# kserve/kserve

Hardware: AMD Instinct MI355X
Metric: output tok/s, llama-3-8b /v1/completions decode (higher is better)
Workload: dtype bfloat16; 1 GPU; model=llama-3-8b, global_batch=1536, seq_len=512, parallelism=dp1, kv_block_size=16, hipgraph=True, kv_cache_dtype=auto

## Files before the change

### kserve_amd/ops/csrc/attention_decode.hip

```cpp
#include "common.h"
#include "mfma_layouts.h"

#define NEG_INF (-1e30f)

namespace {

constexpr int PAGE = 16;
constexpr int NWAVES = 4;

typedef __bf16 bf16x2v_t __attribute__((ext_vector_type(2)));

template <int D, int HPW, int OCC = 1, bool PB = false, bool D2 = false,
          bool V4 = false, bool MQ = false>
__global__ __launch_bounds__(256, OCC) void paged_attention_kernel(
    short* __restrict__ out,
    const short* __restrict__ q,
    const short* __restrict__ k_cache,
    const short* __restrict__ v_cache,
    const int* __restrict__ block_tables,
    const int* __restrict__ context_lens,
    const float scale,
    const int num_kv_heads,
    const int group,
    const int max_blocks,
    const long q_row_stride,
    const int n_splits,
    float* __restrict__ part_out,
    float* __restrict__ part_ml,
    const int window
) {
  constexpr int ACC = D / 64;
  const int kv_head = blockIdx.x;
  const int seq = blockIdx.y;
  const int split = blockIdx.z;
  const int ctx = context_lens[seq];
  if (ctx <= 0) return;
  const int num_heads = num_kv_heads * group;
  const int lane = threadIdx.x & 63;
  const int wave = threadIdx.x >> 6;
  const int tok = lane >> 2;
  const int part = lane & 3;
  __shared__ float p_bc[NWAVES][PAGE];

  const int nblocks = (ctx + PAGE - 1) / PAGE;
  const int wstart = (window > 0 && ctx > window) ? ctx - window : 0;
  const int first_blk = wstart / PAGE;
  const int blocks_per_split =
      (nblocks - first_blk + n_splits - 1) / n_splits;
  const int blk_lo = first_blk + split * blocks_per_split;
  const int blk_hi = min(nblocks, blk_lo + blocks_per_split);
  if (blk_lo >= blk_hi) {
    if (n_splits > 1 && threadIdx.x < (unsigned)group) {
      const int h = kv_head * group + threadIdx.x;
      float* ml = part_ml + (((long)seq * num_heads + h) * n_splits + split) * 2;
      ml[0] = NEG_INF;
      ml[1] = 0.f;
    }
    return;
  }

  constexpr int QFRAG = D / 4;
  float q_frag[HPW][D2 ? 1 : QFRAG];
  bf16x2v_t q_pk[HPW][D2 ? QFRAG / 2 : 1];
  int heads[HPW];
  bool hact[HPW];
  bool any_active = false;
  const int nw = blockDim.x >> 6;
#pragma unroll
  for (int h = 0; h < HPW; ++h) {
    const int head = kv_head * group + wave + h * nw;
    heads[h] = head;
    hact[h] = (wave + h * nw) < group;
    any_active |= hact[h];
    if (hact[h]) {
      const short* qp =
          q + (long)seq * q_row_stride + (long)head * D + part * QFRAG;
      if constexpr (D2) {
        const bf16x2v_t* qp2 = reinterpret_cast<const bf16x2v_t*>(qp);
#pragma unroll
        for (int j = 0; j < QFRAG / 2; ++j) q_pk[h][j] = qp2[j];
      } else {
#pragma unroll
        for (int j = 0; j < QFRAG; ++j)
          q_frag[h][j] = bf16_bits_to_float(qp[j]);
      }
    }
  }

  bf16x8_t q_mf[MQ ? D / 32 : 1];
  if constexpr (MQ) {
    const short* qb = q + (long)seq * q_row_stride + (long)heads[0] * D;
#pragma unroll
    for (int ki = 0; ki < D / 32; ++ki)
      q_mf[ki] = *reinterpret_cast<const bf16x8_t*>(
          qb + ki * 32 + ((lane >> 4) << 3));
  }

  float m[HPW], l[HPW];
  float acc[HPW][ACC];
  float acc8[V4 ? 8 : 1];
#pragma unroll
  for (int h = 0; h < HPW; ++h) {
    m[h] = NEG_INF;
    l[h] = 0.f;
#pragma unroll
    for (int a = 0; a < ACC; ++a) acc[h][a] = 0.f;
  }
#pragma unroll
  for (int a = 0; a < (V4 ? 8 : 1); ++a) acc8[a] = 0.f;

  if (!any_active) return;
  const int bt_base = (int)((long)seq * max_blocks);
  for (int bi = blk_lo; bi < blk_hi; ++bi) {
    const int block_id = block_tables[bt_base + bi];
    const short* page =
        k_cache + (((long)block_id * num_kv_heads + kv_head) * PAGE) * D;
    const short8_t* kp =
        reinterpret_cast<const short8_t*>(page + tok * D + part * QFRAG);
    const int gtok = bi * PAGE + tok;
    const bool tok_valid = gtok < ctx && gtok >= wstart;
    const short* vpage =
        v_cache + (((long)block_id * num_kv_heads + kv_head) * PAGE) * D;

    if constexpr (MQ && HPW == 1 && V4) {
      short8_t vwide4[4];
      const int vdim = (lane & 15) * 8;
      const int vtok4 = lane >> 4;
#pragma unroll
      for (int q4 = 0; q4 < 4; ++q4)
        vwide4[q4] = *reinterpret_cast<const short8_t*>(
            vpage + (q4 * 4 + vtok4) * D + vdim);
      f32x4_t cfrag = f32x4_t{0.f, 0.f, 0.f, 0.f};
#pragma unroll
      for (int ki = 0; ki < D / 32; ++ki) {
        const bf16x8_t bk = *reinterpret_cast<const bf16x8_t*>(
            page + (lane & 15) * D + ki * 32 + ((lane >> 4) << 3));
        cfrag = mfma16x16x32(q_mf[ki], bk, cfrag);
      }
      const int mytok = bi * PAGE + (lane & 15);
      const bool my_valid =
          lane < 16 && mytok < ctx && mytok >= wstart;
      float s = my_valid ? cfrag[0] * scale : NEG_INF;
      float tmax = s;
#pragma unroll
      for (int off = 1; off < 64; off <<= 1)
        tmax = fmaxf(tmax, __shfl_xor(tmax, off, 64));
      const float m_new = fmaxf(m[0], tmax);
      const float rescale = __expf(m[0] - m_new);
      const float p = (s > NEG_INF) ? __expf(s - m_new) : 0.f;
      float psum = p;
#pragma unroll
      for (int off = 1; off < 64; off <<= 1)
        psum += __shfl_xor(psum, off, 64);
      l[0] = l[0] * rescale + psum;
      m[0] = m_new;
      if (lane < 16) p_bc[wave][lane] = p;
      asm volatile("s_waitcnt lgkmcnt(0)");
#pragma unroll
      for (int a = 0; a < 8; ++a) acc8[a] *= rescale;
#pragma unroll
      for (int q4 = 0; q4 < 4; ++q4) {
// ... 563 lines not shown
  const int split = blockIdx.z;
  const int ctx = context_lens[seq];
  if (ctx <= 0) return;
  const int num_heads = num_kv_heads * GROUP;
  const int lane = threadIdx.x & 63;
  const int wave = threadIdx.x >> 6;
  const int tok = lane >> 2;
  const int part = lane & 3;

  const int nblocks = (ctx + PAGE - 1) / PAGE;
  const int wstart = (window > 0 && ctx > window) ? ctx - window : 0;
  const int first_blk = wstart / PAGE;
  const int blocks_per_split =
      (nblocks - first_blk + n_splits - 1) / n_splits;
  const int blk_lo = first_blk + split * blocks_per_split;
  const int blk_hi = min(nblocks, blk_lo + blocks_per_split);

  __shared__ float lds_ml[NWAVES][GROUP][2];
  __shared__ float lds_acc[NWAVES][GROUP][64 * ACC];

  if (blk_lo >= blk_hi) {
    if (n_splits > 1 && threadIdx.x < (unsigned)GROUP) {
      const int h = kv_head * GROUP + threadIdx.x;
      float* ml = part_ml + (((long)seq * num_heads + h) * n_splits + split) * 2;
      ml[0] = NEG_INF;
      ml[1] = 0.f;
    }
    return;
  }

  const short8_t* qrows[GROUP];
#pragma unroll
  for (int g = 0; g < GROUP; ++g) {
    qrows[g] = reinterpret_cast<const short8_t*>(
        q + (long)seq * q_row_stride + (long)(kv_head * GROUP + g) * D +
        part * QFRAG);
  }

  float m[GROUP], l[GROUP], acc[GROUP][ACC];
#pragma unroll
  for (int g = 0; g < GROUP; ++g) {
    m[g] = NEG_INF;
    l[g] = 0.f;
#pragma unroll
    for (int a = 0; a < ACC; ++a) acc[g][a] = 0.f;
  }

  const int bt_base = (int)((long)seq * max_blocks);
  for (int bi = blk_lo + wave; bi < blk_hi; bi += NWAVES) {
    const int block_id = block_tables[bt_base + bi];
    const long pbase = (((long)block_id * num_kv_heads + kv_head) * PAGE) * D;
    const short8_t* kp =
        reinterpret_cast<const short8_t*>(k_cache + pbase + tok * D + part * QFRAG);
    short8_t kreg[QFRAG / 8];
#pragma unroll
    for (int c = 0; c < QFRAG / 8; ++c) kreg[c] = kp[c];
    const short* vpage = v_cache + pbase;
    unsigned int vreg[PAGE];
#pragma unroll
    for (int t = 0; t < PAGE; ++t) {
      if constexpr (ACC == 2) {
        vreg[t] =
            *reinterpret_cast<const unsigned int*>(vpage + t * D + lane * ACC);
      } else {
        vreg[t] = (unsigned short)*(vpage + t * D + lane);
      }
    }
    const int gtok = bi * PAGE + tok;
    const bool tok_valid = gtok < ctx && gtok >= wstart;
#pragma unroll 1
    for (int g = 0; g < GROUP; ++g) {
      float s = 0.f;
#pragma unroll
      for (int c = 0; c < QFRAG / 8; ++c) {
        const short8_t qv = qrows[g][c];
#pragma unroll
        for (int j = 0; j < 8; ++j)
          s += bf16_bits_to_float(qv[j]) * bf16_bits_to_float(kreg[c][j]);
      }
      s = group_reduce_sum<4>(s);
      s = tok_valid ? s * scale : NEG_INF;
      const float tmax = wave_reduce_max(s);
      const float m_new = fmaxf(m[g], tmax);
      const float rescale = __expf(m[g] - m_new);
      const float p = (s > NEG_INF) ? __expf(s - m_new) : 0.f;
      const float psum = wave_reduce_sum(part == 0 ? p : 0.f);
      l[g] = l[g] * rescale + psum;
#pragma unroll
      for (int a = 0; a < ACC; ++a) acc[g][a] *= rescale;
      m[g] = m_new;
#pragma unroll
      for (int t = 0; t < PAGE; ++t) {
        const float pt = __shfl(p, t * 4, 64);
        if constexpr (ACC == 2) {
          acc[g][0] += pt * bf16_bits_to_float((short)(vreg[t] & 0xFFFF));
          acc[g][1] += pt * bf16_bits_to_float((short)(vreg[t] >> 16));
        } else {
          acc[g][0] += pt * bf16_bits_to_float((short)vreg[t]);
        }
      }
    }
  }

#pragma unroll
  for (int g = 0; g < GROUP; ++g) {
    if (lane == 0) {
      lds_ml[wave][g][0] = m[g];
      lds_ml[wave][g][1] = l[g];
    }
#pragma unroll
    for (int a = 0; a < ACC; ++a)
      lds_acc[wave][g][lane * ACC + a] = acc[g][a];
  }
  __syncthreads();
  for (int g = wave; g < GROUP; g += NWAVES) {
    float m_all = NEG_INF;
#pragma unroll
    for (int w = 0; w < NWAVES; ++w) m_all = fmaxf(m_all, lds_ml[w][g][0]);
    float l_all = 0.f;
    float a_all[ACC];
#pragma unroll
    for (int a = 0; a < ACC; ++a) a_all[a] = 0.f;
#pragma unroll
    for (int w = 0; w < NWAVES; ++w) {
      const float wgt = __expf(lds_ml[w][g][0] - m_all);
      l_all += wgt * lds_ml[w][g][1];
#pragma unroll
      for (int a = 0; a < ACC; ++a)
        a_all[a] += wgt * lds_acc[w][g][lane * ACC + a];
    }
    const int head = kv_head * GROUP + g;
    if (n_splits == 1) {
      const float inv_l = (l_all > 0.f) ? 1.f / l_all : 0.f;
      short* op = out + ((long)seq * num_heads + head) * D + lane * ACC;
#pragma unroll
      for (int a = 0; a < ACC; ++a)
        op[a] = float_to_bf16_bits(a_all[a] * inv_l);
    } else {
      float* po = part_out +
                  (((long)seq * num_heads + head) * n_splits + split) * D +
                  lane * ACC;
#pragma unroll
      for (int a = 0; a < ACC; ++a) po[a] = a_all[a];
      if (lane == 0) {
        float* ml =
            part_ml + (((long)seq * num_heads + head) * n_splits + split) * 2;
        ml[0] = m_all;
        ml[1] = l_all;
      }
    }
  }
}

template <int D>
__global__ void paged_attention_reduce_kernel(
    short* __restrict__ out,
    const float* __restrict__ part_out,
    const float* __restrict__ part_ml,
    const long total_sh, const int n_splits) {
  constexpr int ACC = D / 64;
  const long sh = blockIdx.x * (long)(blockDim.x >> 6) + (threadIdx.x >> 6);
  const int lane = threadIdx.x & 63;
  if (sh >= total_sh) return;
  const float* ml_base = part_ml + sh * n_splits * 2;
  float m = NEG_INF;
  for (int sp = 0; sp < n_splits; ++sp) m = fmaxf(m, ml_base[sp * 2]);
  float l = 0.f;
  float acc[ACC];
#pragma unroll
  for (int a = 0; a < ACC; ++a) acc[a] = 0.f;
  for (int sp = 0; sp < n_splits; ++sp) {
    const float ms = ml_base[sp * 2];
    const float ls = ml_base[sp * 2 + 1];
    if (ls <= 0.f || ms <= NEG_INF) continue;
    const float w = __expf(ms - m);
    l += ls * w;
    const float* po = part_out + (sh * n_splits + sp) * D + lane * ACC;
#pragma unroll
    for (int a = 0; a < ACC; ++a) acc[a] += w * po[a];
  }
  const float inv_l = (l > 0.f) ? 1.f / l : 0.f;
  short* op = out + sh * D + lane * ACC;
#pragma unroll
  for (int a = 0; a < ACC; ++a) op[a] = float_to_bf16_bits(acc[a] * inv_l);
}

}


namespace {
inline hipError_t launch_split_reduce(void* out, void* part_out,
                                      void* part_ml, int num_seqs,
                                      int num_heads, int head_dim,
                                      int n_splits, hipStream_t stream) {
  if (n_splits <= 1) return hipSuccess;
  const long sh = (long)num_seqs * num_heads;
  const int wpb = 4;
  dim3 rgrid((unsigned)((sh + wpb - 1) / wpb));
  if (head_dim == 128) {
    hipLaunchKernelGGL((paged_attention_reduce_kernel<128>), rgrid,
                       dim3(wpb * 64), 0, stream, (short*)out,
                       (const float*)part_out, (const float*)part_ml, sh,
                       n_splits);
  } else {
    hipLaunchKernelGGL((paged_attention_reduce_kernel<64>), rgrid,
                       dim3(wpb * 64), 0, stream, (short*)out,
                       (const float*)part_out, (const float*)part_ml, sh,
                       n_splits);
  }
  HIP_CHECK_KERNEL();
  return hipSuccess;
}
}

extern "C" hipError_t ks_paged_attention_decode_fp8(
    void* out, const void* q, const void* k_cache, const void* v_cache,
    const void* block_tables, const void* context_lens, float scale,
    int num_seqs, int num_heads, int num_kv_heads, int head_dim,
    int max_blocks, int block_size, long q_row_stride, int n_splits,
    void* part_out, void* part_ml, int window, hipStream_t stream) {
  if (block_size != PAGE || head_dim != 128) return hipErrorInvalidValue;
  const int group = num_heads / num_kv_heads;
  if (group > NWAVES) return hipErrorInvalidValue;
  if (n_splits < 1) n_splits = 1;
  dim3 grid(num_kv_heads, num_seqs, n_splits);
  static const bool cvtb = [] {
    const char* e = getenv("KS_FP8_CVTB");
    return e == nullptr || e[0] != '0';
  }();
  if (cvtb) {
    hipLaunchKernelGGL((paged_attention_fp8_kernel<128, true>), grid,
                       dim3(256), 0, stream, (short*)out, (const short*)q,
                       (const unsigned char*)k_cache,
                       (const unsigned char*)v_cache,
                       (const int*)block_tables, (const int*)context_lens,
                       scale, num_kv_heads, group, max_blocks, q_row_stride,
                       n_splits, (float*)part_out, (float*)part_ml, window);
  } else {
    hipLaunchKernelGGL((paged_attention_fp8_kernel<128, false>), grid,
                       dim3(256), 0, stream, (short*)out, (const short*)q,
                       (const unsigned char*)k_cache,
                       (const unsigned char*)v_cache,
                       (const int*)block_tables, (const int*)context_lens,
                       scale, num_kv_heads, group, max_blocks, q_row_stride,
                       n_splits, (float*)part_out, (float*)part_ml, window);
  }
  HIP_CHECK_KERNEL();
  return launch_split_reduce(out, part_out, part_ml, num_seqs, num_heads,
                             head_dim, n_splits, stream);
}

extern "C" hipError_t ks_paged_attention_decode(
    void* out, const void* q, const void* k_cache, const void* v_cache,
    const void* block_tables, const void* context_lens, float scale,
    int num_seqs, int num_heads, int num_kv_heads, int head_dim,
    int max_blocks, int block_size, long q_row_stride, int n_splits,
    void* part_out, void* part_ml, int window, hipStream_t stream) {
  if (block_size != PAGE) return hipErrorInvalidValue;
  const int group = num_heads / num_kv_heads;
  const int hpw = (group + NWAVES - 1) / NWAVES;
  if (hpw > 2) return hipErrorInvalidValue;
  if (n_splits < 1) n_splits = 1;
  dim3 grid(num_kv_heads, num_seqs, n_splits);
  dim3 block(256);

  static const bool use_ws = [] {
    const char* e = getenv("KS_ATTN_WS");
    return e != nullptr && e[0] == '1';
  }();
  const bool pow2_group =
      group == 1 || group == 2 || group == 4 || group == 8;
  if (use_ws && pow2_group && head_dim == 128) {
#define LAUNCH_WS(GG)                                                       \
  hipLaunchKernelGGL((paged_attention_ws_kernel<128, GG>), grid, block, 0,  \
                     stream, (short*)out, (const short*)q,                  \
                     (const short*)k_cache, (const short*)v_cache,          \
                     (const int*)block_tables, (const int*)context_lens,    \
                     scale, num_kv_heads, max_blocks, q_row_stride,         \
                     n_splits, (float*)part_out, (float*)part_ml, window)
    if (group == 1) LAUNCH_WS(1);
    else if (group == 2) LAUNCH_WS(2);
    else if (group == 4) LAUNCH_WS(4);
    else LAUNCH_WS(8);
#undef LAUNCH_WS
    HIP_CHECK_KERNEL();
    return launch_split_reduce(out, part_out, part_ml, num_seqs, num_heads,
                               head_dim, n_splits, stream);
  }

  static const bool use_h2 = [] {
    const char* e = getenv("KS_ATTN_H2");
    return e != nullptr && e[0] == '1';
  }();
  if (use_h2 && group == 4 && head_dim == 128) {
    hipLaunchKernelGGL((paged_attention_kernel<128, 2>), grid, dim3(128), 0,
                       stream, (short*)out, (const short*)q,
                       (const short*)k_cache, (const short*)v_cache,
                       (const int*)block_tables, (const int*)context_lens,
                       scale, num_kv_heads, group, max_blocks, q_row_stride,
                       n_splits, (float*)part_out, (float*)part_ml, window);
    HIP_CHECK_KERNEL();
    return launch_split_reduce(out, part_out, part_ml, num_seqs, num_heads,
                               head_dim, n_splits, stream);
  }

  static const bool use_mq = [] {
    const char* e = getenv("KS_ATTN_MQ");
    return e != nullptr && e[0] == '1';
  }();
  if (use_mq && hpw == 1 && head_dim == 128) {
    hipLaunchKernelGGL(
        (paged_attention_kernel<128, 1, 1, true, false, true, true>), grid,
        block, 0, stream, (short*)out, (const short*)q,
        (const short*)k_cache, (const short*)v_cache,
        (const int*)block_tables, (const int*)context_lens, scale,
        num_kv_heads, group, max_blocks, q_row_stride, n_splits,
        (float*)part_out, (float*)part_ml, window);
    HIP_CHECK_KERNEL();
    return launch_split_reduce(out, part_out, part_ml, num_seqs, num_heads,
                               head_dim, n_splits, stream);
  }

  static const bool use_u2 = [] {
    const char* e = getenv("KS_ATTN_U2");
    return e != nullptr && e[0] == '1';
  }();
  if (use_u2 && hpw == 1 && head_dim == 128) {
    hipLaunchKernelGGL((paged_attention_u2_kernel<128>), grid, block, 0,
                       stream, (short*)out, (const short*)q,
                       (const short*)k_cache, (const short*)v_cache,
                       (const int*)block_tables, (const int*)context_lens,
                       scale, num_kv_heads, group, max_blocks, q_row_stride,
                       n_splits, (float*)part_out, (float*)part_ml, window);
    HIP_CHECK_KERNEL();
    return launch_split_reduce(out, part_out, part_ml, num_seqs, num_heads,
                               head_dim, n_splits, stream);
  }
  static const int occ = [] {
    const char* e = getenv("KS_ATTN_OCC");
    return e ? atoi(e) : 0;
  }();
  static const bool use_pb = [] {
    const char* e = getenv("KS_ATTN_PB");
    return e == nullptr || e[0] != '0';
  }();
  static const int v4_mode = [] {
    const char* e = getenv("KS_ATTN_V4");
    return e ? (e[0] == '1' ? 1 : 0) : -1;
  }();
  const bool use_v4 =
      v4_mode == 1 || (v4_mode == -1 && num_seqs > 128);
  static const bool v4_d2 = [] {
    const char* e = getenv("KS_ATTN_V4D2");
    return e != nullptr && e[0] == '1';
  }();
  if (use_v4 && hpw == 1 && head_dim == 128) {
    if (v4_d2) {
      hipLaunchKernelGGL(
          (paged_attention_kernel<128, 1, 1, true, true, true>), grid, block,
          0, stream, (short*)out, (const short*)q, (const short*)k_cache,
          (const short*)v_cache, (const int*)block_tables,
          (const int*)context_lens, scale, num_kv_heads, group, max_blocks,
          q_row_stride, n_splits, (float*)part_out, (float*)part_ml, window);
    } else {
      hipLaunchKernelGGL(
          (paged_attention_kernel<128, 1, 1, true, false, true>), grid,
          block, 0, stream, (short*)out, (const short*)q,
          (const short*)k_cache, (const short*)v_cache,
          (const int*)block_tables, (const int*)context_lens, scale,
          num_kv_heads, group, max_blocks, q_row_stride, n_splits,
          (float*)part_out, (float*)part_ml, window);
    }
    HIP_CHECK_KERNEL();
    return launch_split_reduce(out, part_out, part_ml, num_seqs, num_heads,
                               head_dim, n_splits, stream);
  }
  static const int d2_mode = [] {
    const char* e = getenv("KS_ATTN_D2");
    return e ? (e[0] == '1' ? 1 : 0) : -1;
  }();
  const bool use_d2 =
      d2_mode == 1 || (d2_mode == -1 && num_seqs <= 128);
  if (use_d2 && hpw == 1 && head_dim == 128) {
    hipLaunchKernelGGL((paged_attention_kernel<128, 1, 1, true, true>), grid,
                       block, 0, stream, (short*)out, (const short*)q,
                       (const short*)k_cache, (const short*)v_cache,
                       (const int*)block_tables, (const int*)context_lens,
                       scale, num_kv_heads, group, max_blocks, q_row_stride,
                       n_splits, (float*)part_out, (float*)part_ml, window);
    HIP_CHECK_KERNEL();
    return launch_split_reduce(out, part_out, part_ml, num_seqs, num_heads,
                               head_dim, n_splits, stream);
  }
  if (use_pb && hpw == 1 && head_dim == 128) {
    hipLaunchKernelGGL((paged_attention_kernel<128, 1, 1, true>), grid, block,
                       0, stream, (short*)out, (const short*)q,
                       (const short*)k_cache, (const short*)v_cache,
                       (const int*)block_tables, (const int*)context_lens,
                       scale, num_kv_heads, group, max_blocks, q_row_stride,
                       n_splits, (float*)part_out, (float*)part_ml, window);
    HIP_CHECK_KERNEL();
    return launch_split_reduce(out, part_out, part_ml, num_seqs, num_heads,
                               head_dim, n_splits, stream);
  }
  if (occ >= 5 && hpw == 1 && head_dim == 128) {
    if (occ >= 6) {
      hipLaunchKernelGGL((paged_attention_kernel<128, 1, 6>), grid, block, 0,
                         stream, (short*)out, (const short*)q,
                         (const short*)k_cache, (const short*)v_cache,
                         (const int*)block_tables, (const int*)context_lens,
                         scale, num_kv_heads, group, max_blocks, q_row_stride,
                         n_splits, (float*)part_out, (float*)part_ml, window);
    } else {
      hipLaunchKernelGGL((paged_attention_kernel<128, 1, 5>), grid, block, 0,
                         stream, (short*)out, (const short*)q,
                         (const short*)k_cache, (const short*)v_cache,
                         (const int*)block_tables, (const int*)context_lens,
                         scale, num_kv_heads, group, max_blocks, q_row_stride,
                         n_splits, (float*)part_out, (float*)part_ml, window);
    }
    HIP_CHECK_KERNEL();
    return launch_split_reduce(out, part_out, part_ml, num_seqs, num_heads,
                               head_dim, n_splits, stream);
  }
#define LAUNCH_PA(DD, HH)                                                  \
  hipLaunchKernelGGL((paged_attention_kernel<DD, HH>), grid, block, 0,     \
                     stream, (short*)out, (const short*)q,                 \
                     (const short*)k_cache, (const short*)v_cache,         \
                     (const int*)block_tables, (const int*)context_lens,   \
                     scale, num_kv_heads, group, max_blocks, q_row_stride, \
                     n_splits, (float*)part_out, (float*)part_ml, window)
  if (head_dim == 128) {
    if (hpw == 1) LAUNCH_PA(128, 1);
    else LAUNCH_PA(128, 2);
  } else if (head_dim == 64) {
    if (hpw == 1) LAUNCH_PA(64, 1);
    else LAUNCH_PA(64, 2);
  } else {
    return hipErrorInvalidValue;
  }
#undef LAUNCH_PA
  HIP_CHECK_KERNEL();
  return launch_split_reduce(out, part_out, part_ml, num_seqs, num_heads,
                             head_dim, n_splits, stream);
}
```

### kserve_amd/ops/csrc/bindings.cpp

```cpp
#include <torch/extension.h>

#include <c10/hip/HIPStream.h>

#include <hip/hip_runtime.h>

extern "C" {
hipError_t ks_rms_norm(void*, const void*, const void*, float, int, int,
                       hipStream_t);
hipError_t ks_fused_add_rms_norm(void*, void*, const void*, float, int, int,
                                 hipStream_t);
hipError_t ks_silu_and_mul(void*, const void*, int, int, hipStream_t);
hipError_t ks_rotary_embedding(void*, void*, const void*, const void*, int,
                               int, int, int, long, long, hipStream_t);
hipError_t ks_reshape_and_cache(const void*, const void*, void*, void*,
                                const void*, int, int, int, int, long, long,
                                hipStream_t);
hipError_t ks_paged_attention_decode(void*, const void*, const void*,
                                     const void*, const void*, const void*,
                                     float, int, int, int, int, int, int,
                                     long, int, void*, void*, int,
                                     hipStream_t);
hipError_t ks_flash_prefill_varlen(void*, const void*, const void*,
                                   const void*, const void*, int, int, int,
                                   int, int, float, long, long, long, int,
// ... 6 lines not shown
hipError_t ks_paged_attention_decode_fp8(void*, const void*, const void*,
                                         const void*, const void*,
                                         const void*, float, int, int, int,
                                         int, int, int, long, int, void*,
                                         void*, int, hipStream_t);
hipError_t ks_reshape_and_cache_fp8(const void*, const void*, void*, void*,
                                    const void*, int, int, int, int, long,
                                    long, hipStream_t);
hipError_t ks_layer_norm(void*, const void*, const void*, const void*, float,
                         int, int, hipStream_t);
hipError_t ks_fused_add_layer_norm(void*, const void*, const void*,
                                   const void*, const void*, float, int, int,
                                   hipStream_t);
hipError_t ks_gelu(void*, const void*, long, hipStream_t);
hipError_t ks_greedy_sample(void*, const void*, int, int, hipStream_t);
hipError_t ks_gumbel_sample(void*, const void*, const void*, const void*,
                            const void*, int, int, hipStream_t);
hipError_t ks_topk_topp_sample(void*, const void*, const void*, const void*,
                               const void*, const void*, int, int,
                               hipStream_t);
hipError_t ks_mfma_probe(void*, const void*, const void*, hipStream_t);
hipError_t ks_skinny_gemm(void*, void*, const void*, const void*, int, int,
                          int, long, hipStream_t);
hipError_t ks_gemm8(void*, const void*, const void*, int, int, int, int,
                    hipStream_t);
int ks_skinny_gemm_w8_nsplit(int, int);
hipError_t ks_skinny_gemm_w8(void*, void*, const void*, const void*,
                             const void*, int, int, int, long, hipStream_t);
hipError_t ks_dequant_fp8_rows(void*, const void*, const void*, long, int,
                               hipStream_t);
}

namespace {

hipStream_t current_stream() {
  return c10::hip::getCurrentHIPStream().stream();
}

void check_hip(hipError_t err, const char* op) {
  TORCH_CHECK(err == hipSuccess, op, " failed: ", hipGetErrorString(err));
}

#define CHECK_BF16_CONTIG(t)                                       \
  TORCH_CHECK((t).scalar_type() == at::kBFloat16, #t " must be bf16"); \
  TORCH_CHECK((t).is_contiguous(), #t " must be contiguous");      \
  TORCH_CHECK((t).is_cuda(), #t " must be on GPU")

#define CHECK_KV_CACHE(t)                                               \
  TORCH_CHECK((t).scalar_type() == at::kBFloat16 ||                       \
                  (t).scalar_type() == at::kFloat8_e4m3fn,                \
              #t " must be bf16 or fp8_e4m3");                            \
  TORCH_CHECK((t).is_contiguous(), #t " must be contiguous");             \
  TORCH_CHECK((t).is_cuda(), #t " must be on GPU")

#define CHECK_BF16_ROWS(t)                                              \
  TORCH_CHECK((t).scalar_type() == at::kBFloat16, #t " must be bf16");  \
  TORCH_CHECK((t).is_cuda(), #t " must be on GPU");                     \
  TORCH_CHECK((t).dim() == 3 && (t).stride(2) == 1 &&                   \
                  (t).stride(1) == (t).size(2),                         \
              #t " inner dims must be dense")

void rms_norm(at::Tensor& out, at::Tensor& input, at::Tensor& weight,
              double eps) {
  CHECK_BF16_CONTIG(out);
  CHECK_BF16_CONTIG(input);
  CHECK_BF16_CONTIG(weight);
  int hidden = input.size(-1);
  int rows = input.numel() / hidden;
  check_hip(ks_rms_norm(out.data_ptr(), input.data_ptr(), weight.data_ptr(),
                        (float)eps, rows, hidden, current_stream()),
            "rms_norm");
}

void fused_add_rms_norm(at::Tensor& x, at::Tensor& residual, at::Tensor& weight,
                        double eps) {
  CHECK_BF16_CONTIG(x);
  CHECK_BF16_CONTIG(residual);
  int hidden = x.size(-1);
  int rows = x.numel() / hidden;
  check_hip(
      ks_fused_add_rms_norm(x.data_ptr(), residual.data_ptr(),
                            weight.data_ptr(), (float)eps, rows, hidden,
                            current_stream()),
      "fused_add_rms_norm");
}

void silu_and_mul(at::Tensor& out, at::Tensor& input) {
  CHECK_BF16_CONTIG(out);
  CHECK_BF16_CONTIG(input);
  int d = out.size(-1);
  TORCH_CHECK(input.size(-1) == 2 * d, "input last dim must be 2*out");
  int rows = out.numel() / d;
  check_hip(ks_silu_and_mul(out.data_ptr(), input.data_ptr(), rows, d,
                            current_stream()),
            "silu_and_mul");
}

void rotary_embedding(at::Tensor& positions, at::Tensor& q, at::Tensor& k,
                      at::Tensor& cos_sin_cache) {
  CHECK_BF16_ROWS(q);
  CHECK_BF16_ROWS(k);
  TORCH_CHECK(positions.scalar_type() == at::kLong, "positions must be int64");
  TORCH_CHECK(cos_sin_cache.scalar_type() == at::kFloat,
              "cos_sin_cache must be fp32");
  int T = q.size(0);
  int Hq = q.size(1);
  int Hk = k.size(1);
  int D = q.size(2);
  check_hip(ks_rotary_embedding(q.data_ptr(), k.data_ptr(),
                                positions.data_ptr(), cos_sin_cache.data_ptr(),
                                T, Hq, Hk, D, (long)q.stride(0),
                                (long)k.stride(0), current_stream()),
            "rotary_embedding");
}

void reshape_and_cache(at::Tensor& k, at::Tensor& v, at::Tensor& k_cache,
                       at::Tensor& v_cache, at::Tensor& slot_mapping) {
  CHECK_BF16_ROWS(k);
  CHECK_BF16_ROWS(v);
  CHECK_KV_CACHE(k_cache);
  CHECK_KV_CACHE(v_cache);
  TORCH_CHECK(slot_mapping.scalar_type() == at::kInt, "slot_mapping int32");
  int T = k.size(0);
  int Hkv = k.size(1);
  int D = k.size(2);
  int block_size = k_cache.size(2);
  if (k_cache.scalar_type() == at::kFloat8_e4m3fn) {
    check_hip(ks_reshape_and_cache_fp8(k.data_ptr(), v.data_ptr(),
                                       k_cache.data_ptr(), v_cache.data_ptr(),
                                       slot_mapping.data_ptr(), T, Hkv, D,
                                       block_size, (long)k.stride(0),
                                       (long)v.stride(0), current_stream()),
              "reshape_and_cache_fp8");
    return;
  }
  check_hip(ks_reshape_and_cache(k.data_ptr(), v.data_ptr(),
                                 k_cache.data_ptr(), v_cache.data_ptr(),
                                 slot_mapping.data_ptr(), T, Hkv, D,
                                 block_size, (long)k.stride(0),
                                 (long)v.stride(0), current_stream()),
            "reshape_and_cache");
}

void paged_attention_decode(at::Tensor& out, at::Tensor& q,
                            at::Tensor& k_cache, at::Tensor& v_cache,
                            at::Tensor& block_tables, at::Tensor& context_lens,
                            double scale, int64_t window) {
  CHECK_BF16_CONTIG(out);
  CHECK_BF16_ROWS(q);
  CHECK_KV_CACHE(k_cache);
  CHECK_KV_CACHE(v_cache);
  TORCH_CHECK(block_tables.scalar_type() == at::kInt, "block_tables int32");
  TORCH_CHECK(context_lens.scalar_type() == at::kInt, "context_lens int32");
  const bool fp8 = k_cache.scalar_type() == at::kFloat8_e4m3fn;
  int S = q.size(0);
  int H = q.size(1);
  int D = q.size(2);
  int Hkv = k_cache.size(1);
  int block_size = k_cache.size(2);
  int max_blocks = block_tables.size(1);
  int n_splits = 1;
  long base_wgs = (long)S * Hkv;
  const int grp = H / Hkv;
  static const int split_override = [] {
    const char* e = getenv("KS_ATTN_SPLIT");
    return e ? atoi(e) : 0;
  }();
  if (split_override > 0) {
    n_splits = split_override;
  } else if (grp <= 4 && base_wgs <= 512) {
    n_splits = (int)(2048 / base_wgs);
    if (n_splits < 2) n_splits = 2;
    if (n_splits > 8) n_splits = 8;
  } else if (base_wgs < 512) {
    n_splits = (int)((512 + base_wgs - 1) / base_wgs);
    if (n_splits > 16) n_splits = 16;
  }
  if (n_splits > 1) {
    int max_split_blocks = (max_blocks + n_splits - 1) / n_splits;
    if (max_split_blocks < 1) n_splits = 1;
  }
  at::Tensor part_out, part_ml;
  void *po = nullptr, *pml = nullptr;
  if (n_splits > 1) {
    auto opts = at::TensorOptions().dtype(at::kFloat).device(q.device());
    part_out = at::empty({S, H, n_splits, D}, opts);
    part_ml = at::empty({S, H, n_splits, 2}, opts);
    po = part_out.data_ptr();
    pml = part_ml.data_ptr();
  }
  if (fp8) {
    TORCH_CHECK(H / Hkv <= 4 && D == 128,
                "fp8 KV decode supports D=128 and GQA group <= 4");
    check_hip(ks_paged_attention_decode_fp8(
                  out.data_ptr(), q.data_ptr(), k_cache.data_ptr(),
                  v_cache.data_ptr(), block_tables.data_ptr(),
                  context_lens.data_ptr(), (float)scale, S, H, Hkv, D,
                  max_blocks, block_size, (long)q.stride(0), n_splits, po,
                  pml, (int)window, current_stream()),
              "paged_attention_decode_fp8");
    return;
  }
  check_hip(ks_paged_attention_decode(
                out.data_ptr(), q.data_ptr(), k_cache.data_ptr(),
                v_cache.data_ptr(), block_tables.data_ptr(),
                context_lens.data_ptr(), (float)scale, S, H, Hkv, D,
                max_blocks, block_size, (long)q.stride(0), n_splits, po, pml,
                (int)window, current_stream()),
            "paged_attention_decode");
}

void flash_prefill_varlen(at::Tensor& out, at::Tensor& q, at::Tensor& k,
                          at::Tensor& v, at::Tensor& cu_seqlens,
                          int64_t max_seqlen, double scale,
                          bool causal = true, int64_t window = 0) {
  CHECK_BF16_CONTIG(out);
  CHECK_BF16_ROWS(q);
  CHECK_BF16_ROWS(k);
  CHECK_BF16_ROWS(v);
  TORCH_CHECK(cu_seqlens.scalar_type() == at::kInt, "cu_seqlens int32");
  int num_seqs = cu_seqlens.size(0) - 1;
  int Hq = q.size(1);
  int Hkv = k.size(1);
  int D = q.size(2);
  check_hip(ks_flash_prefill_varlen(out.data_ptr(), q.data_ptr(), k.data_ptr(),
                                    v.data_ptr(), cu_seqlens.data_ptr(),
                                    num_seqs, (int)max_seqlen, Hq, Hkv, D,
                                    (float)scale, (long)q.stride(0),
                                    (long)k.stride(0), (long)v.stride(0),
                                    causal ? 1 : 0, (int)window,
                                    current_stream()),
            "flash_prefill_varlen");
}

void context_prefill_varlen(at::Tensor& out, at::Tensor& q,
                            at::Tensor& k_cache, at::Tensor& v_cache,
                            at::Tensor& block_tables, at::Tensor& ctx_lens,
                            at::Tensor& cu_seqlens_q, int64_t max_q_len,
                            double scale, int64_t window) {
  CHECK_BF16_CONTIG(out);
  CHECK_BF16_ROWS(q);
  CHECK_KV_CACHE(k_cache);
  CHECK_KV_CACHE(v_cache);
  TORCH_CHECK(block_tables.scalar_type() == at::kInt, "block_tables int32");
  TORCH_CHECK(block_tables.is_contiguous(), "block_tables contiguous");
  TORCH_CHECK(ctx_lens.scalar_type() == at::kInt, "ctx_lens int32");
  TORCH_CHECK(cu_seqlens_q.scalar_type() == at::kInt, "cu_seqlens_q int32");
  TORCH_CHECK(k_cache.size(2) == 16, "block_size must be 16");
  int num_seqs = cu_seqlens_q.size(0) - 1;
  int Hq = q.size(1);
  int Hkv = k_cache.size(1);
  int D = q.size(2);
  int fp8 = k_cache.scalar_type() == at::kFloat8_e4m3fn ? 1 : 0;
  check_hip(ks_context_prefill_varlen(
                out.data_ptr(), q.data_ptr(), k_cache.data_ptr(),
                v_cache.data_ptr(), block_tables.data_ptr(),
                ctx_lens.data_ptr(), cu_seqlens_q.data_ptr(), num_seqs,
                (int)max_q_len, Hq, Hkv, D, (int)block_tables.size(1),
                (float)scale, (long)q.stride(0), fp8, (int)window,
                current_stream()),
            "context_prefill_varlen");
}

void layer_norm(at::Tensor& out, at::Tensor& input, at::Tensor& weight,
                at::Tensor& bias, double eps) {
  CHECK_BF16_CONTIG(out);
  CHECK_BF16_CONTIG(input);
  int hidden = input.size(-1);
  int rows = input.numel() / hidden;
  check_hip(ks_layer_norm(out.data_ptr(), input.data_ptr(), weight.data_ptr(),
                          bias.data_ptr(), (float)eps, rows, hidden,
                          current_stream()),
            "layer_norm");
}

void fused_add_layer_norm(at::Tensor& out, at::Tensor& input,
                          at::Tensor& residual, at::Tensor& weight,
                          at::Tensor& bias, double eps) {
  CHECK_BF16_CONTIG(out);
  CHECK_BF16_CONTIG(input);
  CHECK_BF16_CONTIG(residual);
  int hidden = input.size(-1);
  int rows = input.numel() / hidden;
  check_hip(ks_fused_add_layer_norm(out.data_ptr(), input.data_ptr(),
                                    residual.data_ptr(), weight.data_ptr(),
                                    bias.data_ptr(), (float)eps, rows, hidden,
                                    current_stream()),
            "fused_add_layer_norm");
}

void gelu(at::Tensor& out, at::Tensor& input) {
  CHECK_BF16_CONTIG(out);
  CHECK_BF16_CONTIG(input);
  check_hip(ks_gelu(out.data_ptr(), input.data_ptr(), input.numel(),
                    current_stream()),
            "gelu");
}

void greedy_sample(at::Tensor& out, at::Tensor& logits) {
  CHECK_BF16_CONTIG(logits);
  TORCH_CHECK(out.scalar_type() == at::kLong, "out int64");
  check_hip(ks_greedy_sample(out.data_ptr(), logits.data_ptr(),
                             logits.size(0), logits.size(1),
                             current_stream()),
            "greedy_sample");
}
// ... 162 lines not shown
```

Measured before the change: 30080 tok/s.

## Add software-pipelined V4 paged attention decode kernel with double-buffered page loads

Adds a new decode attention kernel for head_dim 128 and one head per wave. It double-buffers K/V page loads in registers so the next page's loads overlap the current page's compute. Cross-lane reductions use DPP and permlane swap builtins, and block table ids are fetched 64 at a time and broadcast with readlane. It becomes the default V4 path, selected for large batches. The risks are higher register pressure and barrier loops for idle waves, plus new contiguity checks on block_tables and context_lens.

```diff
diff --git a/kserve_amd/ops/csrc/attention_decode.hip b/kserve_amd/ops/csrc/attention_decode.hip
--- a/kserve_amd/ops/csrc/attention_decode.hip
+++ b/kserve_amd/ops/csrc/attention_decode.hip
@@ -7,6 +7,7 @@
 
 constexpr int PAGE = 16;
 constexpr int NWAVES = 4;
+constexpr bool V4PIPE_DEFAULT = true;
 
 typedef __bf16 bf16x2v_t __attribute__((ext_vector_type(2)));
 
@@ -876,6 +877,214 @@
   }
 }
 
+template <int CTRL>
+__device__ __forceinline__ float dpp_mov(float v) {
+  return __builtin_bit_cast(
+      float, __builtin_amdgcn_update_dpp(0, __builtin_bit_cast(int, v), CTRL,
+                                         0xf, 0xf, true));
+}
+constexpr int DPP_QUAD_XOR1 = 0xB1;
+constexpr int DPP_QUAD_XOR2 = 0x4E;
+constexpr int DPP_ROW_ROR4 = 0x124;
+constexpr int DPP_ROW_ROR8 = 0x128;
+constexpr int DPP_ROW_MIRROR = 0x140;
+constexpr int DPP_ROW_HALF_MIRROR = 0x141;
+
+__device__ __forceinline__ float rows_max(float v) {
+  const unsigned u = __builtin_bit_cast(unsigned, v);
+  auto r = __builtin_amdgcn_permlane16_swap(u, u, false, false);
+  v = fmaxf(__builtin_bit_cast(float, (unsigned)r[0]),
+            __builtin_bit_cast(float, (unsigned)r[1]));
+  const unsigned w = __builtin_bit_cast(unsigned, v);
+  r = __builtin_amdgcn_permlane32_swap(w, w, false, false);
+  return fmaxf(__builtin_bit_cast(float, (unsigned)r[0]),
+               __builtin_bit_cast(float, (unsigned)r[1]));
+}
+__device__ __forceinline__ float rows_sum(float v) {
+  const unsigned u = __builtin_bit_cast(unsigned, v);
+  auto r = __builtin_amdgcn_permlane16_swap(u, u, false, false);
+  v = __builtin_bit_cast(float, (unsigned)r[0]) +
+      __builtin_bit_cast(float, (unsigned)r[1]);
+  const unsigned w = __builtin_bit_cast(unsigned, v);
+  r = __builtin_amdgcn_permlane32_swap(w, w, false, false);
+  return __builtin_bit_cast(float, (unsigned)r[0]) +
+         __builtin_bit_cast(float, (unsigned)r[1]);
+}
+
+__global__ __launch_bounds__(256) void paged_attention_v4p_kernel(
+    short* __restrict__ out, const short* __restrict__ q,
+    const short* __restrict__ k_cache, const short* __restrict__ v_cache,
+    const int* __restrict__ block_tables, const int* __restrict__ context_lens,
+    const float scale, const int num_kv_heads, const int group,
+    const int max_blocks, const long q_row_stride, const int n_splits,
+    float* __restrict__ part_out, float* __restrict__ part_ml,
+    const int window) {
+  constexpr int D = 128;
+  constexpr int QFRAG = D / 4;
+  const int kv_head = blockIdx.x;
+  const int seq = blockIdx.y;
+  const int split = blockIdx.z;
+  const int ctx = context_lens[seq];
+  if (ctx <= 0) return;
+  const int num_heads = num_kv_heads * group;
+  const int lane = threadIdx.x & 63;
+  const int wave = __builtin_amdgcn_readfirstlane(threadIdx.x >> 6);
+  const int tok = lane >> 2;
+  const int part = lane & 3;
+  const int vtok = lane >> 4;
+  const int vdim = (lane & 15) * 8;
+  __shared__ __attribute__((aligned(16))) float p_bc[NWAVES][PAGE];
+
+  const int nblocks = (ctx + PAGE - 1) / PAGE;
+  const int wstart = (window > 0 && ctx > window) ? ctx - window : 0;
+  const int first_blk = wstart / PAGE;
+  const int blocks_per_split =
+      (nblocks - first_blk + n_splits - 1) / n_splits;
+  const int blk_lo = first_blk + split * blocks_per_split;
+  const int blk_hi = min(nblocks, blk_lo + blocks_per_split);
+  if (blk_lo >= blk_hi) {
+    if (n_splits > 1 && threadIdx.x < (unsigned)group) {
+      const int h = kv_head * group + threadIdx.x;
+      float* ml = part_ml + (((long)seq * num_heads + h) * n_splits + split) * 2;
+      ml[0] = NEG_INF;
+      ml[1] = 0.f;
+    }
+    return;
+  }
+  const int npages = blk_hi - blk_lo;
+  if (wave >= group) {
+    for (int i = 0; i < npages; i += 2) __builtin_amdgcn_s_barrier();
+    return;
+  }
+  const int head = kv_head * group + wave;
+
+  float q_frag[QFRAG];
+  {
+    const short* qp =
+        q + (long)seq * q_row_stride + (long)head * D + part * QFRAG;
+#pragma unroll
+    for (int j = 0; j < QFRAG; ++j) q_frag[j] = bf16_bits_to_float(qp[j]);
+  }
+
+  const int* bt_row = block_tables + (long)seq * max_blocks + blk_lo;
+  auto load_ids = [&](int c0) {
+    return bt_row[min(c0 + lane, npages - 1)];
+  };
+  const int k_off = tok * D + part * QFRAG;
+  const int v_off = vtok * D + vdim;
+  const long head_off = (long)kv_head * PAGE * D;
+  const long blk_stride = (long)num_kv_heads * PAGE * D;
+  auto load_page = [&](int block_id, short8_t* kreg, short8_t* vreg) {
+    const long pbase = (long)block_id * blk_stride + head_off;
+    const short8_t* kp =
+        reinterpret_cast<const short8_t*>(k_cache + pbase + k_off);
+#pragma unroll
+    for (int c = 0; c < 4; ++c) kreg[c] = kp[c];
+    const short* vp = v_cache + pbase + v_off;
+#pragma unroll
+    for (int q4 = 0; q4 < 4; ++q4)
+      vreg[q4] = *reinterpret_cast<const short8_t*>(vp + q4 * 4 * D);
+  };
+
+  float m = NEG_INF;
+  float l = 0.f;
+  float acc8[8];
+#pragma unroll
+  for (int a = 0; a < 8; ++a) acc8[a] = 0.f;
+  float* pw = &p_bc[wave][(tok & 3) * 4 + (tok >> 2)];
+  const float4_t* pr = reinterpret_cast<const float4_t*>(&p_bc[wave][vtok * 4]);
+
+  auto compute_page = [&](int bi, const short8_t* kreg,
+                          const short8_t* vreg) {
+#pragma clang fp reassociate(off)
+    float lo = 0.f, hi = 0.f;
+#pragma unroll
+    for (int i = 0; i < 16; ++i) {
+      const int r = i & 3, g = i >> 2;
+      const int c = r == 0 ? 1 : (r == 1 ? 0 : r);
+      const int w = g == 0 ? 2 : (g == 1 ? 0 : (g == 2 ? 3 : 1));
+      const float kl = bf16_bits_to_float(kreg[c][2 * w]);
+      const float kh = bf16_bits_to_float(kreg[c][2 * w + 1]);
+      const float ql = q_frag[c * 8 + 2 * w], qh = q_frag[c * 8 + 2 * w + 1];
+      lo = i == 0 ? ql * kl : __builtin_fmaf(ql, kl, lo);
+      hi = i == 0 ? qh * kh : __builtin_fmaf(qh, kh, hi);
+    }
+    float s = lo + hi;
+    s += dpp_mov<DPP_QUAD_XOR2>(s);
+    s += dpp_mov<DPP_QUAD_XOR1>(s);
+    const int gtok = bi * PAGE + tok;
+    s = (gtok < ctx && gtok >= wstart) ? s * scale : NEG_INF;
+    float tmax = fmaxf(s, dpp_mov<DPP_ROW_ROR4>(s));
+    tmax = fmaxf(tmax, dpp_mov<DPP_ROW_ROR8>(tmax));
+    tmax = rows_max(tmax);
+    const float m_new = fmaxf(m, tmax);
+    const float rescale = __expf(m - m_new);
+    const float p = (s > NEG_INF) ? __expf(s - m_new) : 0.f;
+    float psum = p + dpp_mov<DPP_ROW_HALF_MIRROR>(p);
+    psum += dpp_mov<DPP_ROW_MIRROR>(psum);
+    psum = rows_sum(psum);
+    l = __builtin_fmaf(l, rescale, psum);
+    m = m_new;
+    __builtin_amdgcn_fence(__ATOMIC_RELEASE, "wavefront");
+    if (part == 0) *pw = p;
+    __builtin_amdgcn_fence(__ATOMIC_SEQ_CST, "wavefront");
+    const float4_t pt4 = *pr;
+    __builtin_amdgcn_fence(__ATOMIC_ACQUIRE, "wavefront");
+#pragma unroll
+    for (int a = 0; a < 8; ++a) acc8[a] *= rescale;
+#pragma unroll
+    for (int q4 = 0; q4 < 4; ++q4) {
+      const float pt = pt4[q4];
+#pragma unroll
+      for (int a = 0; a < 8; ++a)
+        acc8[a] = __builtin_fmaf(pt, bf16_bits_to_float(vreg[q4][a]), acc8[a]);
+    }
+  };
+
+  short8_t kA[4], vA[4], kB[4], vB[4];
+  int ids_next = load_ids(0);
+  load_page(__builtin_amdgcn_readlane(ids_next, 0), kA, vA);
+  for (int c0 = 0; c0 < npages; c0 += 64) {
+    const int ids = ids_next;
+    ids_next = load_ids(c0 + 64);
+    const int cn = min(64, npages - c0);
+    for (int j = 0; j < cn; j += 2) {
+      __builtin_amdgcn_s_barrier();
+      load_page(__builtin_amdgcn_readlane(ids, min(j + 1, cn - 1)), kB, vB);
+      compute_page(blk_lo + c0 + j, kA, vA);
+      const int id_a = __builtin_amdgcn_readlane(ids, min(j + 2, cn - 1));
+      const int id_n = __builtin_amdgcn_readlane(ids_next, 0);
+      load_page(j + 2 < 64 ? id_a : id_n, kA, vA);
+      if (j + 1 < cn) compute_page(blk_lo + c0 + j + 1, kB, vB);
+    }
+  }
+
+#pragma unroll
+  for (int a = 0; a < 8; ++a) acc8[a] = rows_sum(acc8[a]);
+  if (n_splits == 1) {
+    const float inv_l = (l > 0.f) ? 1.f / l : 0.f;
+    if (lane < 16) {
+      short* op = out + ((long)seq * num_heads + head) * D + vdim;
+#pragma unroll
+      for (int a = 0; a < 8; ++a) op[a] = float_to_bf16_bits(acc8[a] * inv_l);
+    }
+  } else {
+    if (lane < 16) {
+      float* po = part_out +
+                  (((long)seq * num_heads + head) * n_splits + split) * D +
+                  vdim;
+#pragma unroll
+      for (int a = 0; a < 8; ++a) po[a] = acc8[a];
+    }
+    if (lane == 0) {
+      float* ml =
+          part_ml + (((long)seq * num_heads + head) * n_splits + split) * 2;
+      ml[0] = m;
+      ml[1] = l;
+    }
+  }
+}
+
 template <int D>
 __global__ void paged_attention_reduce_kernel(
     short* __restrict__ out,
@@ -1078,8 +1287,19 @@
     const char* e = getenv("KS_ATTN_V4D2");
     return e != nullptr && e[0] == '1';
   }();
+  static const bool v4_pipe = [] {
+    const char* e = getenv("KS_ATTN_V4PIPE");
+    return e ? e[0] == '1' : V4PIPE_DEFAULT;
+  }();
   if (use_v4 && hpw == 1 && head_dim == 128) {
-    if (v4_d2) {
+    if (v4_pipe && !v4_d2) {
+      hipLaunchKernelGGL(
+          paged_attention_v4p_kernel, grid, block, 0, stream, (short*)out,
+          (const short*)q, (const short*)k_cache, (const short*)v_cache,
+          (const int*)block_tables, (const int*)context_lens, scale,
+          num_kv_heads, group, max_blocks, q_row_stride, n_splits,
+          (float*)part_out, (float*)part_ml, window);
+    } else if (v4_d2) {
       hipLaunchKernelGGL(
           (paged_attention_kernel<128, 1, 1, true, true, true>), grid, block,
           0, stream, (short*)out, (const short*)q, (const short*)k_cache,
diff --git a/kserve_amd/ops/csrc/bindings.cpp b/kserve_amd/ops/csrc/bindings.cpp
--- a/kserve_amd/ops/csrc/bindings.cpp
+++ b/kserve_amd/ops/csrc/bindings.cpp
@@ -182,6 +182,8 @@
   CHECK_KV_CACHE(v_cache);
   TORCH_CHECK(block_tables.scalar_type() == at::kInt, "block_tables int32");
   TORCH_CHECK(context_lens.scalar_type() == at::kInt, "context_lens int32");
+  TORCH_CHECK(block_tables.is_contiguous(), "block_tables must be contiguous");
+  TORCH_CHECK(context_lens.is_contiguous(), "context_lens must be contiguous");
   const bool fp8 = k_cache.scalar_type() == at::kFloat8_e4m3fn;
   int S = q.size(0);
   int H = q.size(1);
```

New measurement: 30660 tok/s, median of 6. +1.9%, better.
